# hanmekim/SceneLib2

Measured on NVIDIA H100. Metric: EKF-SLAM frames/sec @320x240 N=100 feats, higher is better.
Workload: dtype f64 (EKF, scores) + u8/int32 (correlation sums)

## Files before the change

scenelib2_b200/csrc/update.cu:

```cuda
#include <type_traits>

#include "sl2_context.cuh"
#include "sl2_ptx.cuh"

using namespace sl2;

namespace {

constexpr int UPD_THREADS = 256;
constexpr int UPD_NB = 16;
constexpr int UPD_WS = 20;
constexpr int UPD_DS = 20;
constexpr int UPD_MS = 20;
constexpr int UPD_YS = 68;
constexpr int SOLVE_MAX_WARPS = 8;

__host__ __device__ inline int upd_keven(int kmax) { return (kmax + 1) & ~1; }
__host__ __device__ inline int upd_panw(int kmax) {
  return ((2 * upd_keven(kmax) + 15) & ~15) + 2;
}
__host__ __device__ inline size_t upd_pan_doubles(int kmax) { return (size_t)UPD_NB * upd_panw(kmax); }

__device__ __forceinline__ void dmma884(double &c0, double &c1, double a, double b) {
  asm("mma.sync.aligned.m8n8k4.row.col.f64.f64.f64.f64 {%0,%1}, {%2}, {%3}, {%0,%1};"
// ... 627 lines not shown
        const double *gpre = G + (size_t)lc * ldg + n0 + lr;
        double *mp = mnext + lc * UPD_MS + lr;
        const bool v0 = lr < nbn, v1 = 8 + lr < nbn;
        auto loadv = [&](double *dst) {
          const double x0 = gpre[0], x1 = gpre[8];
          dst[0] = v0 ? -x0 : 0.0;
          dst[1] = v1 ? -x1 : 0.0;
          gpre += kstride;
        };
        auto step = [&](const double *vu) {
          const double a[2] = {vu[0], vu[1]};
          mp[0] = a[0];
          mp[8] = a[1];
          mp += 4 * UPD_MS;
          dmma1684(c[0], a, -a[0]);
          dmma1684(c[1], a, -a[1]);
        };
#pragma unroll
        for (int u = 0; u < CH_D - 1; ++u)
          if (u < nk) loadv(v[u]);
        int kb = 0;
        for (; kb + CH_D <= nk; kb += CH_D) {
#pragma unroll
          for (int u = 0; u < CH_D; ++u) {
            if (kb + u + CH_D - 1 < nk) loadv(v[(u + CH_D - 1) % CH_D]);
            step(v[u]);
          }
        }
#pragma unroll
        for (int q = 0; q < 2; ++q)
#pragma unroll
          for (int mt = 0; mt < 2; ++mt)
            *reinterpret_cast<double2 *>(dnext + (mt * 8 + lr) * CH_DPS + 8 * q + 2 * lc) =
                make_double2(c[q][2 * mt], c[q][2 * mt + 1]);
      } else {
        const int bt = it - 2;
        if (gb == 4) chol_batch<4, 4>(G, ldg, mcur, sm.pan, PW, i0, nbp, nk, ngroups, width, 2 + bt * 4, lr, lc);
        else if (gb == 2) chol_batch<2, 8>(G, ldg, mcur, sm.pan, PW, i0, nbp, nk, ngroups, width, 2 + bt * 2, lr, lc);
        else chol_batch<1, 8>(G, ldg, mcur, sm.pan, PW, i0, nbp, nk, ngroups, width, 2 + bt, lr, lc);
      }
    }
    __syncthreads();
    const int ncol = width - i0;
    for (int e = tid; e < UPD_NB * UPD_NB; e += UPD_THREADS) {
      const int r = e / UPD_NB, cc = e - r * UPD_NB;
      if (r < nbp && cc < nbp && i0 + cc < width)
        G[(size_t)(i0 + r) * ldg + i0 + cc] = (cc >= r) ? sm.dg[r * UPD_DS + cc] : 0.0;
      Wp[(size_t)pidx * 256 + e] = sm.Wm[r * UPD_WS + cc];
      if (r >= nbp || UPD_NB + cc >= ncol) mnext[(i0 + r) * UPD_MS + cc] = 0.0;
    }
    if (tid == 0) s_next = 1;
    {
      double aw[4][2];
#pragma unroll
      for (int mt = 0; mt < 2; ++mt)
#pragma unroll
        for (int ks = 0; ks < 4; ++ks) aw[ks][mt] = sm.Wm[(mt * 8 + lr) * UPD_WS + 4 * ks + lc];
      constexpr int FG = 4;
      for (int gb = 2 + warp; gb * 8 < ncol; gb += FG * (UPD_THREADS / 32)) {
        double c[FG][4];
#pragma unroll
        for (int f = 0; f < FG; ++f) c[f][0] = c[f][1] = c[f][2] = c[f][3] = 0.0;
#pragma unroll
        for (int ks = 0; ks < 4; ++ks) {
          double bv[FG];
#pragma unroll
          for (int f = 0; f < FG; ++f) {
            const int cb = (gb + f * (UPD_THREADS / 32)) * 8 + lr;
            bv[f] = cb < ncol ? sm.pan[(size_t)(4 * ks + lc) * PW + cb] : 0.0;
          }
#pragma unroll
          for (int f = 0; f < FG; ++f) dmma1684(c[f], aw[ks], bv[f]);
        }
#pragma unroll
        for (int f = 0; f < FG; ++f) {
          const int gq = gb + f * (UPD_THREADS / 32);
          const int cc = gq * 8 + 2 * lc;
#pragma unroll
          for (int mt = 0; mt < 2; ++mt) {
            const int r = mt * 8 + lr;
            if (r < nbp && cc < ncol) {
              double *dst = G + (size_t)(i0 + r) * ldg + i0 + cc;
              if (cc + 1 < ncol) *reinterpret_cast<double2 *>(dst) = make_double2(c[f][2 * mt], c[f][2 * mt + 1]);
              else *dst = c[f][2 * mt];
              if (gq < 4) {
                mnext[(i0 + r) * UPD_MS + cc - UPD_NB] = -c[f][2 * mt];
                if (cc + 1 < ncol) mnext[(i0 + r) * UPD_MS + cc + 1 - UPD_NB] = -c[f][2 * mt + 1];
              }
            }
          }
        }
      }
    }
    __syncthreads();
  }
}

__device__ __forceinline__ double c_to_b(const double (&c)[2][2], int ks, int lane) {
  const int lr = lane >> 2, lc = lane & 3;
  const int src = ((4 * (ks & 1) + lc) << 2) | (lr >> 1);
  const double v0 = __shfl_sync(0xffffffffu, c[ks >> 1][0], src);
  const double v1 = __shfl_sync(0xffffffffu, c[ks >> 1][1], src);
  return (lr & 1) ? v1 : v0;
}

template <int NP> struct SolveLayout {
  static constexpr int SPLIT = NP > 13 ? 6 : NP;
  static constexpr int REUSE = NP > 13 ? 4 : NP;
  __host__ __device__ static constexpr int pw(int p) { return 16 * (NP - 1 - p) + 4; }
  __host__ __device__ static constexpr int off_lin(int p0, int p) {
    int o = 0;
    for (int q = p0; q < p; ++q) o += 16 * pw(q);
    return o;
  }
  __host__ __device__ static constexpr int off(int p) { return p < SPLIT ? off_lin(0, p) : off_lin(SPLIT, p); }
  static constexpr int PAN_DOUBLES = off_lin(0, SPLIT < NP - 1 ? SPLIT : NP - 1);
  static constexpr int SMEM_DOUBLES = PAN_DOUBLES + NP * 16 * UPD_WS + NP + (NP & 1) +
                                      2 * SOLVE_MAX_WARPS * 2 * 32 * 2 +
                                      SOLVE_MAX_WARPS * 128;
  static_assert(SPLIT == NP || off_lin(SPLIT, NP - 1) <= off_lin(0, REUSE), "second generation must fit");
};

template <int NP>
__global__ void __launch_bounds__(64 * SOLVE_MAX_WARPS, 1) upd_solve_kernel(const Sl2Dev d, int stream_lo) {
  using L = SolveLayout<NP>;
  extern __shared__ __align__(16) uint8_t smem_raw[];
  pdl_prologue();
  double *pan = reinterpret_cast<double *>(smem_raw);
  double *Wm = pan + L::PAN_DOUBLES;
  const uint32_t bars = smem_u32(Wm + NP * 16 * UPD_WS);
  double2 *xbuf = reinterpret_cast<double2 *>(Wm + NP * 16 * UPD_WS + NP + (NP & 1));
  double *ybuf = reinterpret_cast<double *>(xbuf + 2 * SOLVE_MAX_WARPS * 2 * 32);
  const int s = stream_lo + blockIdx.y;
  const int m = d.upd_m[s];
  if (m == 0) return;
  const int tid = threadIdx.x, nthr = blockDim.x;
  const int ngrp = nthr >> 6;
  const int warp = tid >> 5, lane = tid & 31, lr = lane >> 2, lc = lane & 3;
  const int g = warp % ngrp, rho = warp / ngrp;
  const int n = SL2_NXV + 3 * d.nfeat[s];
  const int ncols = n + 1;
  if (blockIdx.x * ngrp * 8 >= ncols) return;
  const int ldg = d.ldg;
  double *__restrict__ G = d.G + (size_t)s * d.mmax * ldg;
  const double *__restrict__ Wp = d.Wp + (size_t)s * SL2_MAX_PANELS * 256;
  const int m8 = (m + 7) & ~7;
  const bool full = L::SPLIT == NP && m8 >= 16 * NP - 8;
  const int zend = full ? 16 * NP : m8;

  if (tid == 0) {
    for (int p = 0; p < NP; ++p) mbar_init(bars + 8 * p, 1);
    fence_barrier_init();
    fence_proxy_async();
  }
  auto zero_pads = [&](int plo, int phi) {
    for (int e = tid; e < (phi - plo) * 16; e += nthr) {
      const int p = plo + (e >> 4), r = e & 15;
      const int cfirst = 16 * p + 16;
      if (16 * p < m)
        for (int c = max(m, cfirst); c < zend; ++c) pan[L::off(p) + r * L::pw(p) + (c - cfirst)] = 0.0;
    }
  };
  zero_pads(0, L::SPLIT);
  __syncthreads();
  auto request = [&](int p) {
    if (16 * p < m) {
      const int cfirst = 16 * p + 16;
      const int nrow = min(16, m - 16 * p);
      const uint32_t ubytes = m > cfirst ? (uint32_t)(m - cfirst) * 8u : 0u;
      const uint32_t bar = bars + 8 * p;
      if (lane == 0) mbar_expect_tx(bar, (uint32_t)nrow * ubytes + 16u * 128u);
      __syncwarp();
      if (lane < 16) {
        if (lane < nrow && ubytes)
          bulk_g2s(pan + L::off(p) + lane * L::pw(p), G + (size_t)(16 * p + lane) * ldg + cfirst, ubytes, bar);
      } else {
        bulk_g2s(Wm + ((size_t)p * 16 + (lane - 16)) * UPD_WS, Wp + (size_t)p * 256 + (lane - 16) * 16, 128u, bar);
      }
    }
  };
  if (warp == 0) {
#pragma unroll 1
    for (int p = 0; p < L::SPLIT; ++p) request(p);
  }

  int xpar = 0;
  auto solve_group = [&](auto full_c, const int grp) {
    constexpr bool FULL = decltype(full_c)::value;
    const int c0 = 8 * grp;
    const bool wact = c0 < ncols;
    const int cc = c0 + 2 * lc;
    const int cval = wact ? min(2, ncols - cc) : 0;
    double *gcol = G + m + cc;
    double acc[(NP + 1) & ~1][2];
    {
      const int ccn = cc + 8 * (int)(gridDim.x * ngrp);
      if (L::SPLIT >= NP && ccn < ncols) {
#pragma unroll
        for (int t = 0; t < NP; ++t) {
          const int row = 8 * (2 * t + rho) + lr;
          if (row < m) asm volatile("prefetch.global.L2 [%0];" ::"l"(G + m + ccn + (size_t)row * ldg));
        }
      }
    }
#pragma unroll
    for (int t = 0; t < ((NP + 1) & ~1); ++t) {
      const int row = 8 * (2 * t + rho) + lr;
      acc[t][0] = acc[t][1] = 0.0;
      if (row < m) {
        if (cval >= 2) {
          const double2 v = *reinterpret_cast<const double2 *>(gcol + (size_t)row * ldg);
          acc[t][0] = v.x;
          acc[t][1] = v.y;
        } else if (cval == 1) {
          acc[t][0] = gcol[(size_t)row * ldg];
        }
      }
    }

#pragma unroll
    for (int p = 0; p < NP; ++p) {
      if (FULL || 16 * p < m) {
        if (L::SPLIT < NP && p == L::REUSE) {
          __syncthreads();
          zero_pads(L::SPLIT, NP);
          __syncthreads();
          if (warp == 0) {
            fence_proxy_async();
#pragma unroll 1
            for (int q = L::SPLIT; q < NP; ++q) request(q);
          }
        }
        if (!wact) continue;
        xpar ^= 1;
        double2 *xb = xbuf + ((size_t)(xpar * ngrp + g) * 2) * 32;
        xb[rho * 32 + lane] = make_double2(acc[p][0], acc[p][1]);
        asm volatile("bar.sync %0, 64;" ::"r"(1 + g) : "memory");
        const double2 other = xb[(rho ^ 1) * 32 + lane];
        const double cp2[2][2] = {{rho ? other.x : acc[p][0], rho ? other.y : acc[p][1]},
                                  {rho ? acc[p][0] : other.x, rho ? acc[p][1] : other.y}};
        mbar_wait(bars + 8 * p, 0);
        const double *pb = pan + L::off(p);
        const int PW = L::pw(p);
        const double *wb = Wm + (size_t)p * 16 * UPD_WS;
        double cb[4];
#pragma unroll
        for (int ks = 0; ks < 4; ++ks) cb[ks] = c_to_b(cp2, ks, lane);
        double d0 = 0.0, d1 = 0.0;
#pragma unroll
        for (int ks = 0; ks < 4; ++ks) dmma884(d0, d1, wb[(8 * rho + lr) * UPD_WS + 4 * ks + lc], cb[ks]);
        {
          const int row = 16 * p + 8 * rho + lr;
          if (row < m) {
            if (cval >= 2) *reinterpret_cast<double2 *>(gcol + (size_t)row * ldg) = make_double2(d0, d1);
            else if (cval == 1) gcol[(size_t)row * ldg] = d0;
          }
        }
        if (p + 1 < NP) {
          double *yg = ybuf + (size_t)g * 128;
          *reinterpret_cast<double2 *>(yg + (8 * rho + lr) * 8 + 2 * lc) = make_double2(d0, d1);
          asm volatile("bar.sync %0, 64;" ::"r"(1 + g) : "memory");
          double yb[4];
#pragma unroll
          for (int ks = 0; ks < 4; ++ks) yb[ks] = -yg[(4 * ks + lc) * 8 + lr];
          const double *pbr = pb + 8 * rho + lr;
#pragma unroll
          for (int ks = 0; ks < 4; ++ks) {
#pragma unroll
            for (int t = (p + 1) & ~1; t < NP; t += 2) {
              const bool has[2] = {t > p && (FULL || 8 * (2 * t + rho) < m),
                                   t + 1 < NP && (FULL || 8 * (2 * t + 2 + rho) < m)};
              if (has[0] || has[1]) {
                double a[2];
#pragma unroll
                for (int h = 0; h < 2; ++h) a[h] = has[h] ? pbr[(4 * ks + lc) * PW + 16 * (t + h - p - 1)] : 0.0;
                double c[4] = {acc[t][0], acc[t][1], acc[t + 1][0], acc[t + 1][1]};
                dmma1684(c, a, yb[ks]);
                acc[t][0] = c[0];
                acc[t][1] = c[1];
                acc[t + 1][0] = c[2];
                acc[t + 1][1] = c[3];
              }
            }
          }
        }
      }
    }
  };
  for (int grp = blockIdx.x * ngrp + g; L::SPLIT < NP ? grp == (int)(blockIdx.x * ngrp + g) : 8 * grp < ncols;
       grp += gridDim.x * ngrp) {
    if (L::SPLIT == NP && full) solve_group(std::true_type{}, grp);
    else solve_group(std::false_type{}, grp);
  }
}

constexpr int SYRK_THREADS = 128;
template <int KC, int ST>
__global__ void __launch_bounds__(SYRK_THREADS, 3) upd_syrk_kernel(const Sl2Dev d, int stream_lo) {
  constexpr int STAGE = 2 * KC * UPD_YS;
  constexpr int NW = SYRK_THREADS / 32;
  extern __shared__ __align__(16) uint8_t smem_raw[];
  double *stage_buf = reinterpret_cast<double *>(smem_raw);
  pdl_prologue();
  const int s = stream_lo + blockIdx.y;
  const int m = d.upd_m[s];
  if (m == 0) return;
  const int n = SL2_NXV + 3 * d.nfeat[s];
  int tb = 0;
  const int t = blockIdx.x;
  while ((tb + 1) * (tb + 2) / 2 <= t) ++tb;
  const int ta = t - tb * (tb + 1) / 2;
  if (tb * 64 >= n + 1) return;
  const int tid = threadIdx.x, warp = tid >> 5, lane = tid & 31, lr = lane >> 2, lc = lane & 3;
  const int wa = (warp & 1) * 32, wb = (warp >> 1) * 32;
  const int ld = d.ld, ldg = d.ldg;
  double *__restrict__ P = d.P + (size_t)s * ld * ld;
  double *__restrict__ x = d.x + (size_t)s * ld;
  const double *__restrict__ G = d.G + (size_t)s * d.mmax * ldg;
  const bool diag = ta == tb;
  const int bi0 = wa >> 3, bj0 = wb >> 3;
  unsigned cmask = 0xFFFFu, mmask = 0xFFFFu;
  if (diag) {
    cmask = mmask = 0u;
#pragma unroll
    for (int bi = 0; bi < 4; ++bi)
#pragma unroll
      for (int bj = 0; bj < 4; ++bj) {
        if (bi0 + bi <= bj0 + bj) cmask |= 1u << (4 * bi + bj);
        if (bi0 + bi < bj0 + bj) mmask |= 1u << (4 * bi + bj);
      }
  }
  const bool skip = cmask == 0u;
  if (!skip) {
#pragma unroll
    for (int i = 0; i < 4; ++i) {
      const int a = ta * 64 + wa + i * 8, bq = tb * 64 + wb + lane;
      if (a < n && bq < n) asm volatile("prefetch.global.L2 [%0];" ::"l"(P + a + (size_t)ld * bq));
    }
  }
  const int kr = m, lim = m + n + 1;
  const int nchunk = (kr + KC - 1) / KC;
  const int cA = m + ta * 64 + 2 * lane, cB = m + tb * 64 + 2 * lane;
  const int bytesA = cA + 1 < lim ? 16 : (cA < lim ? 8 : 0);
  const int bytesB = cB + 1 < lim ? 16 : (cB < lim ? 8 : 0);
  const double *srcA = G + (bytesA ? cA : 0);
  const double *srcB = G + (bytesB ? cB : 0);
  const double *pa = srcA + (size_t)warp * ldg, *pb = srcB + (size_t)warp * ldg;
  const uint32_t sdst = smem_u32(stage_buf + 2 * lane + warp * UPD_YS);
  const size_t rstep = (size_t)NW * ldg;
  auto stage = [&](int chunk) {
    const uint32_t dd = sdst + (uint32_t)(chunk % ST) * (STAGE * 8);
    if ((chunk + 1) * KC <= kr) {
#pragma unroll
      for (int j = 0; j < KC / NW; ++j) {
        asm volatile("cp.async.cg.shared.global [%0], [%1], 16, %2;" ::"r"(dd + j * NW * UPD_YS * 8),
                     "l"(pa + j * rstep), "r"(bytesA)
                     : "memory");
        if (!diag)
          asm volatile("cp.async.cg.shared.global [%0], [%1], 16, %2;" ::"r"(dd + (KC + j * NW) * UPD_YS * 8),
                       "l"(pb + j * rstep), "r"(bytesB)
                       : "memory");
      }
    } else {
#pragma unroll
      for (int j = 0; j < KC / NW; ++j) {
        const bool kv = chunk * KC + warp + NW * j < kr;
        asm volatile("cp.async.cg.shared.global [%0], [%1], 16, %2;" ::"r"(dd + j * NW * UPD_YS * 8),
                     "l"(kv ? pa + j * rstep : srcA), "r"(kv ? bytesA : 0)
                     : "memory");
        if (!diag)
          asm volatile("cp.async.cg.shared.global [%0], [%1], 16, %2;" ::"r"(dd + (KC + j * NW) * UPD_YS * 8),
                       "l"(kv ? pb + j * rstep : srcB), "r"(kv ? bytesB : 0)
                       : "memory");
      }
    }
    pa += (size_t)KC * ldg;
    pb += (size_t)KC * ldg;
  };
  double acc[2][4][4];
#pragma unroll
  for (int i = 0; i < 2; ++i)
#pragma unroll
    for (int j = 0; j < 4; ++j)
#pragma unroll
      for (int e = 0; e < 4; ++e) acc[i][j][e] = 0.0;
#pragma unroll
  for (int c = 0; c < ST - 1; ++c) {
    if (c < nchunk) stage(c);
    cp_async_commit();
  }
  for (int ch = 0; ch < nchunk; ++ch) {
    cp_async_wait<ST - 2>();
    __syncthreads();
    if (ch + ST - 1 < nchunk) stage(ch + ST - 1);
    cp_async_commit();
    if (!skip) {
      const double *Ya = stage_buf + (size_t)(ch % ST) * STAGE;
      const double *Yb = diag ? Ya : Ya + KC * UPD_YS;
      const int krem = kr - ch * KC;
      auto chunk = [&](auto diag_c) {
        constexpr bool DIAG = decltype(diag_c)::value;
        auto kstep = [&](int kk) {
          double a[2][4], b[4][2];
#pragma unroll
          for (int i = 0; i < 2; ++i)
#pragma unroll
            for (int e = 0; e < 4; ++e)
              a[i][e] = Ya[(kk + lc + 4 * (e >> 1)) * UPD_YS + wa + 16 * i + 8 * (e & 1) + lr];
#pragma unroll
          for (int j = 0; j < 4; ++j)
#pragma unroll
            for (int e = 0; e < 2; ++e) b[j][e] = Yb[(kk + lc + 4 * e) * UPD_YS + wb + j * 8 + lr];
#pragma unroll
          for (int i = 0; i < 2; ++i)
#pragma unroll
            for (int j = 0; j < 4; ++j)
              if (!DIAG || 2 * i <= j) dmma1688(acc[i][j], a[i], b[j]);
        };
        if (krem >= KC) {
#pragma unroll
          for (int kk = 0; kk < KC; kk += 8) kstep(kk);
        } else {
#pragma unroll 1
          for (int kk = 0; kk < krem; kk += 8) kstep(kk);
        }
      };
      if (cmask == 0xFFFFu) chunk(std::false_type{});
      else chunk(std::true_type{});
    }
  }
  if (skip) return;
#pragma unroll
  for (int bi = 0; bi < 4; ++bi) {
    const int i = bi >> 1, h = bi & 1;
    const int a = ta * 64 + wa + bi * 8 + lr;
    double pold[4][2];
#pragma unroll
    for (int j = 0; j < 4; ++j)
#pragma unroll
      for (int e = 0; e < 2; ++e) {
        const int bq = tb * 64 + wb + j * 8 + 2 * lc + e;
        pold[j][e] = (((cmask >> (4 * bi + j)) & 1u) && a < n && bq < n) ? P[a + (size_t)ld * bq] : 0.0;
      }
#pragma unroll
    for (int j = 0; j < 4; ++j) {
      if (!((cmask >> (4 * bi + j)) & 1u)) continue;
      const int bq = tb * 64 + wb + j * 8 + 2 * lc;
      const double c0 = acc[i][j][2 * h], c1 = acc[i][j][2 * h + 1];
      const double v0 = pold[j][0] - c0, v1 = pold[j][1] - c1;
      if (a < n && bq < n) {
        P[a + (size_t)ld * bq] = v0;
        if (bq + 1 < n) P[a + (size_t)ld * (bq + 1)] = v1;
        if ((mmask >> (4 * bi + j)) & 1u) {
          double *dst = P + bq + (size_t)ld * a;
          if (bq + 1 < n) *reinterpret_cast<double2 *>(dst) = make_double2(v0, v1);
          else *dst = v0;
        }
      }
      if (a < n) {
        if (bq == n) x[a] += c0;
        if (bq + 1 == n) x[a] += c1;
      }
    }
  }
}

__global__ void __launch_bounds__(UPD_THREADS) upd_finish_kernel(const Sl2Dev d, int stream_lo, int staged,
                                                                  int only_normalise, int rescued) {
  pdl_prologue();
  const int s = stream_lo + blockIdx.x;
  const int tid = threadIdx.x;
  const int nf = d.nfeat[s];
  const int n = SL2_NXV + 3 * nf;
  const int ld = d.ld;
  double *__restrict__ P = d.P + (size_t)s * ld * ld;
  const double *__restrict__ x = d.x + (size_t)s * ld;
  const size_t fb = (size_t)s * d.Nmax;
  const int m = only_normalise ? 0 : d.upd_m[s];
  if (rescued && m == 0) return;
  __shared__ int s_cull;
  if (m > 0 || only_normalise) {
    __shared__ double J4[16];
    if (tid == 0) {
      const rd q[4] = {rd(x[3]), rd(x[4]), rd(x[5]), rd(x[6])};
      const rd qq = q[0] * q[0] + q[1] * q[1] + q[2] * q[2] + q[3] * q[3];
      for (int i = 0; i < 4; ++i)
        for (int j = 0; j < 4; ++j)
          J4[i * 4 + j] = (i == j) ? ((rd(1.0) - q[i] * q[i] / (qq * qq)) / qq).v
                                   : ((-q[i]) * q[j] / (qq * qq * qq)).v;
    }
    __syncthreads();
    for (int j = tid; j < n; j += UPD_THREADS) {
      double v[4], o[4];
      for (int k = 0; k < 4; ++k) v[k] = P[(3 + k) + (size_t)ld * j];
      for (int i = 0; i < 4; ++i) {
        rd a(0.0);
        for (int k = 0; k < 4; ++k) a = a + rd(J4[i * 4 + k]) * rd(v[k]);
        o[i] = a.v;
      }
      for (int k = 0; k < 4; ++k) P[(3 + k) + (size_t)ld * j] = o[k];
    }
    __syncthreads();
    for (int i = tid; i < n; i += UPD_THREADS) {
      if (i < SL2_NXV) {
        double v[4], o[4];
        for (int k = 0; k < 4; ++k) v[k] = P[i + (size_t)ld * (3 + k)];
        for (int c = 0; c < 4; ++c) {
          rd a(0.0);
          for (int k = 0; k < 4; ++k) a = a + rd(v[k]) * rd(J4[c * 4 + k]);
          o[c] = a.v;
        }
        for (int k = 0; k < 4; ++k) P[i + (size_t)ld * (3 + k)] = o[k];
      } else {
        for (int k = 0; k < 4; ++k) P[i + (size_t)ld * (3 + k)] = P[(3 + k) + (size_t)ld * i];
      }
    }
    __syncthreads();
  }
  {
    const int i = tid % 13, j = (tid / 13) % 13;
    const double a = P[i + (size_t)ld * j], b = P[j + (size_t)ld * i];
    const double v = (rd(a) * rd(0.5) + rd(b) * rd(0.5)).v;
    __syncthreads();
    if (tid < 169) P[i + (size_t)ld * j] = v;
    __syncthreads();
  }
  if (!staged && !only_normalise) {
    if (tid == 0) s_cull = 0;
    __syncthreads();
    for (int i = tid; i < nf; i += UPD_THREADS) {
      int att = d.attempted[fb + i], suc = d.successful[fb + i];
      if (rescued) {
        if (d.found[fb + i] == SL2_FOUND_RESCUED) {
          suc += 1;
          d.successful[fb + i] = suc;
          d.found[fb + i] = 1;
        }
      } else if (d.sel_rank[fb + i] >= 0) {
        att += 1;
        if (d.found[fb + i] == 1) suc += 1;
        d.attempted[fb + i] = att;
        d.successful[fb + i] = suc;
      }
      if (att >= d.min_attempts && (double)suc / (double)att < d.match_fraction) atomicAdd(&s_cull, 1);
    }
    __syncthreads();
    if (tid == 0) d.ncull[s] = s_cull;
  }
}

struct SolveKernel {
  void (*kern)(Sl2Dev, int);
  int np;
  size_t smem;
};
template <int NP>
SolveKernel solve_kernel_np() {
  return {upd_solve_kernel<NP>, NP, SolveLayout<NP>::SMEM_DOUBLES * sizeof(double)};
}
inline SolveKernel solve_kernel(int kmax) {
  const int p = (2 * upd_keven(kmax) + 15) / 16;
  return p <= 4 ? solve_kernel_np<4>()
                : (p <= 7 ? solve_kernel_np<7>()
                          : (p <= 10 ? solve_kernel_np<10>() : (p <= 13 ? solve_kernel_np<13>() : solve_kernel_np<16>())));
}
inline void solve_shape(int Nmax, int &nslab, int &warps) {
  const int ngroups = (SL2_NXV + 3 * Nmax + 1 + 7) / 8;
  nslab = (ngroups + SOLVE_MAX_WARPS - 1) / SOLVE_MAX_WARPS;
  warps = (ngroups + nslab - 1) / nslab;
}
constexpr size_t SYRK_SMEM = (size_t)2 * 2 * 32 * UPD_YS * sizeof(double);

size_t sl2_update_smem_bytes(const Sl2Dev &d) {
  return chol_smem_doubles(d.kmax) * sizeof(double);
}

}

cudaError_t sl2_configure_update(const Sl2Dev &d) {
  const SolveKernel solve = solve_kernel(d.kmax);
  const struct {
    const void *kern;
    size_t smem;
  } opt_in[] = {
      {(const void *)upd_hp_kernel<7>, hp_layout(d.kmax, d.ld, 0).bytes},
      {(const void *)upd_hp_kernel<13>, hp_layout(d.kmax, d.ld, 0).bytes},
      {(const void *)upd_hp2_kernel<7>, hp_layout(d.kmax, d.ld, 7).bytes},
      {(const void *)upd_hp2_kernel<13>, hp_layout(d.kmax, d.ld, 13).bytes},
      {(const void *)upd_chol_kernel, sl2_update_smem_bytes(d)},
      {(const void *)solve.kern, solve.smem},
      {(const void *)upd_syrk_kernel<32, 2>, SYRK_SMEM},
  };
  for (const auto &k : opt_in) {
    const cudaError_t e = cudaFuncSetAttribute(k.kern, cudaFuncAttributeMaxDynamicSharedMemorySize, (int)k.smem);
    if (e != cudaSuccess) return e;
  }
  return cudaSuccess;
}

namespace {

cudaError_t launch_hp(const Sl2Dev &d, int stream_lo, int stream_cnt, int row_found, int staged_m, const int *st_feat,
                      const double *st_Hxv, const double *st_Hy, const double *st_R, const double *st_nu,
                      const Sl2Subpix &sp, const Sl2Iter &it, Sl2Queue q) {
  const int hp_all = (2 * upd_keven(d.kmax) + HP_ROWS - 1) / HP_ROWS;
  const int hp_blocks = stream_cnt >= 2 * d.nsm ? 1 : hp_all;
  const dim3 grid(hp_blocks, stream_cnt);
  const bool piped = hp_blocks == 1 && SL2_NXV + 3 * d.Nmax <= HP_THREADS;
  const int kd = staged_m >= 0 ? 13 : 7;
  auto *k13 = piped ? upd_hp2_kernel<13> : upd_hp_kernel<13>;
  auto *k7 = piped ? upd_hp2_kernel<7> : upd_hp_kernel<7>;
  const size_t smem = hp_layout(d.kmax, d.ld, piped ? kd : 0).bytes;
  return sl2_launch_kernel(kd == 13 ? k13 : k7, grid, dim3(HP_THREADS), smem, q, sl2_use_pdl(stream_cnt), d, stream_lo,
                           row_found, staged_m, st_feat, st_Hxv, st_Hy, st_R, st_nu, sp, it);
}

cudaError_t launch_chol(const Sl2Dev &d, int stream_lo, int stream_cnt, Sl2Queue q) {
  return sl2_launch_kernel(upd_chol_kernel, dim3(stream_cnt), dim3(UPD_THREADS), sl2_update_smem_bytes(d), q,
                           sl2_use_pdl(stream_cnt), d, stream_lo);
}

cudaError_t launch_update(const Sl2Dev &d, int stream_lo, int stream_cnt, int row_found, int staged_m,
                          const int *st_feat, const double *st_Hxv, const double *st_Hy, const double *st_R,
                          const double *st_nu, int only_normalise, const Sl2Subpix &sp, const Sl2Iter &it, Sl2Queue q,
                          cudaEvent_t *ev6) {
  if (stream_cnt <= 0) return cudaSuccess;
  cudaError_t e;
  auto mark = [&](int i) { return ev6 ? cudaEventRecord(ev6[i], q.stream) : cudaSuccess; };
  if ((e = mark(0)) != cudaSuccess) return e;
  const bool pdl = sl2_use_pdl(stream_cnt);
  if (!only_normalise) {
    e = launch_hp(d, stream_lo, stream_cnt, row_found, staged_m, st_feat, st_Hxv, st_Hy, st_R, st_nu, sp, it, q);
    if (e != cudaSuccess) return e;
  }
  if ((e = mark(1)) != cudaSuccess) return e;
  if (!only_normalise) {
    e = launch_chol(d, stream_lo, stream_cnt, q);
    if (e != cudaSuccess) return e;
  }
  if ((e = mark(2)) != cudaSuccess) return e;
  if (!only_normalise) {
    int nslab, warps;
    solve_shape(d.Nmax, nslab, warps);
    const SolveKernel solve = solve_kernel(d.kmax);
    const bool walk = solve.np <= 13 && stream_cnt >= d.nsm;
    if (walk) warps = SOLVE_MAX_WARPS;
    e = sl2_launch_kernel(solve.kern, dim3(walk ? 1 : nslab, stream_cnt), dim3(64 * warps), solve.smem, q, pdl, d,
                          stream_lo);
    if (e != cudaSuccess) return e;
  }
  if ((e = mark(3)) != cudaSuccess) return e;
  if (!only_normalise) {
    const int nt = (SL2_NXV + 3 * d.Nmax + 1 + 63) / 64;
    e = sl2_launch_kernel(upd_syrk_kernel<32, 2>, dim3(nt * (nt + 1) / 2, stream_cnt), dim3(SYRK_THREADS), SYRK_SMEM,
                          q, pdl, d, stream_lo);
    if (e != cudaSuccess) return e;
  }
  if ((e = mark(4)) != cudaSuccess) return e;
  e = sl2_launch_kernel(upd_finish_kernel, dim3(stream_cnt), dim3(UPD_THREADS), 0, q, pdl, d, stream_lo,
                        (int)(staged_m >= 0), only_normalise, (int)(row_found == SL2_FOUND_RESCUED));
  if (e != cudaSuccess) return e;
  if ((e = mark(5)) != cudaSuccess) return e;
  return cudaGetLastError();
}

}

cudaError_t sl2_launch_update(const Sl2Dev &d, int stream_lo, int stream_cnt, int staged_m,
                              const int *st_feat, const double *st_Hxv, const double *st_Hy,
                              const double *st_R, const double *st_nu, int only_normalise,
                              const Sl2Subpix &sp, Sl2Queue q, cudaEvent_t *ev6, const Sl2Iter &it) {
  return launch_update(d, stream_lo, stream_cnt, 1, staged_m, st_feat, st_Hxv, st_Hy, st_R, st_nu, only_normalise, sp,
                       it, q, ev6);
}

cudaError_t sl2_launch_iterate_factor(const Sl2Dev &d, int stream_lo, int stream_cnt, const Sl2Subpix &sp,
                                      const Sl2Iter &it, Sl2Queue q) {
  if (stream_cnt <= 0) return cudaSuccess;
  cudaError_t e = launch_hp(d, stream_lo, stream_cnt, 1, -1, nullptr, nullptr, nullptr, nullptr, nullptr, sp, it, q);
  if (e != cudaSuccess) return e;
  return launch_chol(d, stream_lo, stream_cnt, q);
}

cudaError_t sl2_launch_update_rescued(const Sl2Dev &d, int stream_lo, int stream_cnt, int *m2, const Sl2Subpix &sp,
                                      Sl2Queue q) {
  Sl2Dev d2 = d;
  d2.upd_m = m2;
  return launch_update(d2, stream_lo, stream_cnt, SL2_FOUND_RESCUED, -1, nullptr, nullptr, nullptr, nullptr, nullptr, 0,
                       sp, Sl2Iter{}, q, nullptr);
}

extern "C" {

int sl2_ekf_update(sl2_ctx *c, int32_t s, int32_t m, const int32_t *feat_index, const double *H_xv,
                   const double *H_y, const double *R, const double *nu) {
  if (bad_stream(c, s) || m < 0 || (m & 1) || m > c->d.mmax)
    return fail(c, SL2_ERR_ARG, "sl2_ekf_update: bad m");
  if (m == 0) return SL2_OK;
  if (!feat_index || !H_xv || !H_y || !R || !nu) return fail(c, SL2_ERR_ARG, "sl2_ekf_update: null argument");
  const int K = m / 2;
  int nf = 0;
  int rc = device_nfeat(c, s, &nf);
  if (rc) return rc;
  for (int k = 0; k < K; ++k) {
    if (feat_index[k] < 0 || feat_index[k] >= nf) return fail(c, SL2_ERR_ARG, "sl2_ekf_update: bad feature index");
    if (R[k * 4 + 1] != R[k * 4 + 2]) return fail(c, SL2_ERR_ARG, "sl2_ekf_update: R block is not symmetric");
  }
  const size_t k = K;
  Stage hx{STAGE_IN, 8 * 26 * k, H_xv}, hy{STAGE_IN, 8 * 6 * k, H_y}, r{STAGE_IN, 8 * 4 * k, R},
      v{STAGE_IN, 8 * 2 * k, nu}, fe{STAGE_IN, 4 * k, feat_index};
  return staged_call(c, {&hx, &hy, &r, &v, &fe}, [] {}, [&] {
    CU_TRY(c, sl2_launch_update(c->d, s, 1, m, fe.dev<int>(), hx.dev<double>(), hy.dev<double>(), r.dev<double>(),
                                v.dev<double>(), 0, Sl2Subpix{}, queue(c)));
    return SL2_OK;
  });
}

int sl2_ekf_update_measured(sl2_ctx *c, int32_t s) {
  if (bad_stream(c, s)) return fail(c, SL2_ERR_ARG, "bad stream");
  const int rc0 = iterate_streams(c, s, 1, queue(c));
  if (rc0) return rc0;
  CU_TRY(c, sl2_launch_update(c->d, s, 1, -1, nullptr, nullptr, nullptr, nullptr, nullptr, 0, subpixel_args(c, s, 1),
                              queue(c), nullptr, iterate_args(c, s, 1)));
  if (rescue_on(c, s, 1)) {
    const int rc = rescue_streams(c, s, 1, queue(c));
    if (rc) return rc;
  }
  CU_TRY(c, cudaStreamSynchronize(c->stream));
  return SL2_OK;
}

int sl2_normalise_state(sl2_ctx *c, int32_t s) {
  if (bad_stream(c, s)) return fail(c, SL2_ERR_ARG, "bad stream");
  CU_TRY(c, sl2_launch_update(c->d, s, 1, -1, nullptr, nullptr, nullptr, nullptr, nullptr, 1, Sl2Subpix{}, queue(c)));
  CU_TRY(c, cudaStreamSynchronize(c->stream));
  return SL2_OK;
}

}
```

Measured before the change: 232,800.

## Balance diagonal SYRK tile work across warps and batch P epilogue loads

On diagonal tiles, warp 1 previously had no work (cmask zero), so it was removed from the compute path. Warps 1 and 2 now each take half of the upper-right 32x32 sub-block, which spreads the tensor-core MMAs more evenly. The epilogue loads all old P values up front, so the global loads overlap instead of being serialized per row block. Streams are also visited in reverse blockIdx.y order. The trade-off is higher register pressure from the 32-double pold array, plus extra code specialization.

```diff
diff --git a/scenelib2_b200/csrc/update.cu b/scenelib2_b200/csrc/update.cu
--- a/scenelib2_b200/csrc/update.cu
+++ b/scenelib2_b200/csrc/update.cu
@@ -953,7 +953,7 @@
   extern __shared__ __align__(16) uint8_t smem_raw[];
   double *stage_buf = reinterpret_cast<double *>(smem_raw);
   pdl_prologue();
-  const int s = stream_lo + blockIdx.y;
+  const int s = stream_lo + (int)(gridDim.y - 1 - blockIdx.y);
   const int m = d.upd_m[s];
   if (m == 0) return;
   const int n = SL2_NXV + 3 * d.nfeat[s];
@@ -963,12 +963,13 @@
   const int ta = t - tb * (tb + 1) / 2;
   if (tb * 64 >= n + 1) return;
   const int tid = threadIdx.x, warp = tid >> 5, lane = tid & 31, lr = lane >> 2, lc = lane & 3;
-  const int wa = (warp & 1) * 32, wb = (warp >> 1) * 32;
+  const bool diag = ta == tb;
+  const bool half = diag && (warp == 1 || warp == 2);
+  const int wa = half ? 0 : (warp & 1) * 32, wb = half ? 32 : (warp >> 1) * 32;
   const int ld = d.ld, ldg = d.ldg;
   double *__restrict__ P = d.P + (size_t)s * ld * ld;
   double *__restrict__ x = d.x + (size_t)s * ld;
   const double *__restrict__ G = d.G + (size_t)s * d.mmax * ldg;
-  const bool diag = ta == tb;
   const int bi0 = wa >> 3, bj0 = wb >> 3;
   unsigned cmask = 0xFFFFu, mmask = 0xFFFFu;
   if (diag) {
@@ -980,14 +981,16 @@
         if (bi0 + bi <= bj0 + bj) cmask |= 1u << (4 * bi + bj);
         if (bi0 + bi < bj0 + bj) mmask |= 1u << (4 * bi + bj);
       }
-  }
-  const bool skip = cmask == 0u;
-  if (!skip) {
-#pragma unroll
-    for (int i = 0; i < 4; ++i) {
-      const int a = ta * 64 + wa + i * 8, bq = tb * 64 + wb + lane;
-      if (a < n && bq < n) asm volatile("prefetch.global.L2 [%0];" ::"l"(P + a + (size_t)ld * bq));
-    }
+    if (half) {
+      cmask &= warp == 2 ? 0x00FFu : 0xFF00u;
+      mmask &= cmask;
+    }
+  }
+#pragma unroll
+  for (int i = 0; i < 4; ++i) {
+    const int a = ta * 64 + wa + i * 8, bq = tb * 64 + wb + lane;
+    if (((cmask >> (4 * i)) & 0xFu) && a < n && bq < n)
+      asm volatile("prefetch.global.L2 [%0];" ::"l"(P + a + (size_t)ld * bq));
   }
   const int kr = m, lim = m + n + 1;
   const int nchunk = (kr + KC - 1) / KC;
@@ -1045,12 +1048,13 @@
     __syncthreads();
     if (ch + ST - 1 < nchunk) stage(ch + ST - 1);
     cp_async_commit();
-    if (!skip) {
+    {
       const double *Ya = stage_buf + (size_t)(ch % ST) * STAGE;
       const double *Yb = diag ? Ya : Ya + KC * UPD_YS;
       const int krem = kr - ch * KC;
-      auto chunk = [&](auto diag_c) {
-        constexpr bool DIAG = decltype(diag_c)::value;
+      auto chunk = [&](auto shape_c) {
+        constexpr int SHAPE = decltype(shape_c)::value;
+        auto issued = [](int i, int j) { return SHAPE == 0 || (SHAPE == 1 ? 2 * i <= j : i == SHAPE - 2); };
         auto kstep = [&](int kk) {
           double a[2][4], b[4][2];
 #pragma unroll
@@ -1066,7 +1070,7 @@
           for (int i = 0; i < 2; ++i)
 #pragma unroll
             for (int j = 0; j < 4; ++j)
-              if (!DIAG || 2 * i <= j) dmma1688(acc[i][j], a[i], b[j]);
+              if (issued(i, j)) dmma1688(acc[i][j], a[i], b[j]);
         };
         if (krem >= KC) {
 #pragma unroll
@@ -1076,29 +1080,37 @@
           for (int kk = 0; kk < krem; kk += 8) kstep(kk);
         }
       };
-      if (cmask == 0xFFFFu) chunk(std::false_type{});
-      else chunk(std::true_type{});
-    }
-  }
-  if (skip) return;
+      if (cmask == 0xFFFFu) chunk(std::integral_constant<int, 0>{});
+      else if (cmask == 0x00FFu) chunk(std::integral_constant<int, 2>{});
+      else if (cmask == 0xFF00u) chunk(std::integral_constant<int, 3>{});
+      else chunk(std::integral_constant<int, 1>{});
+    }
+  }
+  double pold[4][4][2];
+  {
+    const int a0 = ta * 64 + wa + lr, b0 = tb * 64 + wb + 2 * lc;
+    const double *pw = P + a0 + (size_t)ld * b0;
+#pragma unroll
+    for (int j = 0; j < 4; ++j)
+#pragma unroll
+      for (int e = 0; e < 2; ++e) {
+        const double *pc = pw + (size_t)ld * (8 * j + e);
+        const bool bv = b0 + 8 * j + e < n;
+#pragma unroll
+        for (int bi = 0; bi < 4; ++bi)
+          pold[bi][j][e] = (((cmask >> (4 * bi + j)) & 1u) && bv && a0 + 8 * bi < n) ? pc[8 * bi] : 0.0;
+      }
+  }
 #pragma unroll
   for (int bi = 0; bi < 4; ++bi) {
     const int i = bi >> 1, h = bi & 1;
     const int a = ta * 64 + wa + bi * 8 + lr;
-    double pold[4][2];
-#pragma unroll
-    for (int j = 0; j < 4; ++j)
-#pragma unroll
-      for (int e = 0; e < 2; ++e) {
-        const int bq = tb * 64 + wb + j * 8 + 2 * lc + e;
-        pold[j][e] = (((cmask >> (4 * bi + j)) & 1u) && a < n && bq < n) ? P[a + (size_t)ld * bq] : 0.0;
-      }
 #pragma unroll
     for (int j = 0; j < 4; ++j) {
       if (!((cmask >> (4 * bi + j)) & 1u)) continue;
       const int bq = tb * 64 + wb + j * 8 + 2 * lc;
       const double c0 = acc[i][j][2 * h], c1 = acc[i][j][2 * h + 1];
-      const double v0 = pold[j][0] - c0, v1 = pold[j][1] - c1;
+      const double v0 = pold[bi][j][0] - c0, v1 = pold[bi][j][1] - c1;
       if (a < n && bq < n) {
         P[a + (size_t)ld * bq] = v0;
         if (bq + 1 < n) P[a + (size_t)ld * (bq + 1)] = v1;
```

New measurement: 235,000 (median of 6 runs). No clear change (+1.0%).
